# aayush9400/3D-Condtional-Stable-Diffusion

Measured on AMD Instinct MI355X. Metric: latent volumes/sec at 32^3x8ch T=1000 DDPM, higher is better.
Workload: dtype f32 (f16 hi+lo x3 MFMA, f32 accumulate)

## Files before the change

### 3d-condtional-stable-diffusion_amd/csrc/dm3d_conv.hip

```cpp
#include <algorithm>
#include <cstdlib>
#include "dm3d_conv_args.h"
#include <math.h>

namespace {

template <int TD, int TH, int TW, int S, int KS, int WM, int WN>
__global__ __launch_bounds__(256, 2) void conv3d_igemm_f32(const ConvArgs p) {
    constexpr int CK = 16, LDV = CK + 4, NT = 64;
    constexpr int TM = TD * TH * TW;
    constexpr int HD = (TD - 1) * S + KS, HH = (TH - 1) * S + KS, HW = (TW - 1) * S + KS;
    constexpr int HVOX = HD * HH * HW;
    constexpr int TAPS = KS * KS * KS;
    constexpr int MR = TM / WM / 32, NR = NT / WN / 32;
    constexpr int NTHR = WM * WN * 64;
    constexpr int NSLOT = (HVOX * 4 + NTHR - 1) / NTHR;
    static_assert(NTHR == 256, "kernel assumes 4 waves");
    static_assert(TM % (WM * 32) == 0 && NT % (WN * 32) == 0, "tile split");

    extern __shared__ __attribute__((aligned(16))) float smem[];
    float* lds_in = smem;
    float* lds_w = smem + HVOX * LDV;

    const int tid = threadIdx.x;
// ... 97 lines not shown
        for (int tap = 0; tap < TAPS; ++tap) {
            const bool last_tap = tap + 1 == TAPS;
            {
                int nt = tap + 1, nc = c0;
                if (last_tap) { nt = 0; nc = (ch + 1 < p.nchunks) ? c0 + CK : c0; }
                wreg = *reinterpret_cast<const f32x4*>(w_thread + (size_t)nt * w_tap_stride + nc);
            }

            const int kd = tap / (KS * KS), kh = (tap / KS) % KS, kw = tap % KS;
            const int tap_off = ((kd * HH + kh) * HW + kw) * LDV;
            const float* wbuf = lds_w + (tap & 1) * (NT * LDV);
            const float* a_lds[MR];
            const float* b_lds[NR];
#pragma unroll
            for (int mr = 0; mr < MR; ++mr) a_lds[mr] = a_base[mr] + tap_off;
#pragma unroll
            for (int nr = 0; nr < NR; ++nr) b_lds[nr] = wbuf + b_off[nr];
            dm3d_mma_step<MR, NR, CK>(acc, a_lds, b_lds, half);

            if (!last_tap) {
                *reinterpret_cast<f32x4*>(lds_w + ((tap + 1) & 1) * (NT * LDV) + w_lds_off) = wreg;
                __syncthreads();
            }
        }
    }

    const int vrow = p.vec ? (p.vec_idx ? p.vec_idx[b] : b) : 0;
    const size_t sample_elems = (size_t)p.fd * p.fh * p.fw * p.cout;
#pragma unroll
    for (int nr = 0; nr < NR; ++nr) {
        const int n = n0 + wn * (NT / WN) + nr * 32 + l32;
        const bool n_ok = n < p.cout;
        const int nc = n_ok ? n : p.cout - 1;
        float add = p.bias ? p.bias[nc] : 0.0f;
        if (p.vec) add += p.vec[(size_t)vrow * p.vec_ld + nc];
#pragma unroll
        for (int mr = 0; mr < MR; ++mr) {
            size_t o[16];
            bool ok[16];
            float rv[16];
#pragma unroll
            for (int r = 0; r < 16; ++r) {
                const int row = wm * (TM / WM) + mr * 32 + dm3d_acc_row(r, half);
                const int oz = oz0 + row / (TH * TW), oy = oy0 + (row / TW) % TH, ox = ox0 + row % TW;
                ok[r] = n_ok && oz < p.od && oy < p.oh && ox < p.ow;
                o[r] = ok[r] ? ((((size_t)b * p.fd + oz * p.os + ooz) * p.fh + oy * p.os + ooy) * p.fw + ox * p.os + oox) * p.cout + n : 0;
            }
            if (p.res) {
#pragma unroll
                for (int r = 0; r < 16; ++r) rv[r] = p.res[o[r]];
            }
#pragma unroll
            for (int r = 0; r < 16; ++r) {
                float v = acc[mr][nr][r] + add;
                if (p.relu) v = fmaxf(v, 0.0f);
                if (p.prelu) { const float al = p.prelu[o[r] % sample_elems]; v = v > 0.0f ? v : al * v; }
                if (p.res) v += rv[r];
                if (p.relu_out) v = fmaxf(v, 0.0f);
                if (ok[r]) p.out[o[r]] = v;
            }
        }
    }
}

template <int TD, int TH, int TW, int S, int KS, int WM, int WN>
int launch_conv(ConvArgs& a, hipStream_t st) {
    constexpr int LDV = 20;
    constexpr int HVOX = ((TD - 1) * S + KS) * ((TH - 1) * S + KS) * ((TW - 1) * S + KS);
    constexpr size_t lds = (size_t)(HVOX * LDV + 2 * 64 * LDV) * sizeof(float);
    a.bd = (a.od + TD - 1) / TD;
    a.bh = (a.oh + TH - 1) / TH;
    a.bw = (a.ow + TW - 1) / TW;
    static std::atomic<bool> attr_set[64] = {};
    if (int dev = dm3d_dyn_lds(lds, attr_set, "conv", &conv3d_igemm_f32<TD, TH, TW, S, KS, WM, WN>); dev < 0) return dev;
    dim3 grid((unsigned)(a.batch * a.bd * a.bh * a.bw), (unsigned)(a.coutpad / 64), a.parity ? 8u : 1u);
    hipLaunchKernelGGL((conv3d_igemm_f32<TD, TH, TW, S, KS, WM, WN>), grid, dim3(256), lds, st, a);
    return dm3d_launch_check("conv3d_igemm_f32");
}

}


struct ConvKnobs {
    bool pair_off; int ksplit_mode; long split_wgs, split_target; int split_minchunks, split_maxparts; bool wino_split_off;
    int v3_td; long wide_wgs; bool wino_off; int wino_minchunks, wino_split_minchunks;
};
static ConvKnobs conv_knobs() {
    auto num = [](const char* name, long dflt) { const char* e = getenv(name); return e ? atol(e) : dflt; };
    auto zero = [](const char* name) { const char* e = getenv(name); return e && e[0] == '0'; };
    static const ConvKnobs once = {
        zero("DM3D_CONV_PAIR"),
        (int)num("DM3D_CONV_KSPLIT", -1),
        num("DM3D_CONV_SPLIT_WGS", 256),
        num("DM3D_CONV_SPLIT_TARGET", 512),
        (int)num("DM3D_CONV_SPLIT_MINCHUNKS", 2),
        (int)num("DM3D_CONV_SPLIT_MAXPARTS", 16),
        zero("DM3D_CONV_WINO_SPLIT"),
        0, 0, false, 0, 0};
    ConvKnobs k = once;
    k.v3_td = (int)num("DM3D_CONV_V3_TD", 0);
    k.wide_wgs = num("DM3D_CONV_WIDE_WGS", 512);
    k.wino_off = zero("DM3D_CONV_WINO");
    k.wino_minchunks = (int)num("DM3D_CONV_WINO_MINCHUNKS", 2);
    k.wino_split_minchunks = (int)num("DM3D_CONV_WINO_SPLIT_MINCHUNKS", 16);
    return k;
}

static long split_tiles(const ConvArgs& a, int td) {
    return (long)a.batch * ((a.od + td - 1) / td) * ((a.oh + 7) / 8) * ((a.ow + 7) / 8) * (a.coutpad / 64) * (a.parity ? 8 : 1);
}

static int direct_ksplit(const ConvArgs& a, const ConvKnobs& K) {
    const long wgs = split_tiles(a, 4);
    if (K.ksplit_mode == 0 || wgs > K.split_wgs || a.nchunks < 4) return 1;
    int best = 1;
    for (int d = 2; d <= K.split_maxparts; ++d) {
        if (a.nchunks % d != 0 || a.nchunks / d < K.split_minchunks) continue;
        best = d;
        if (wgs * d >= K.split_target) break;
    }
    return best;
}

static int winograd_ksplit(const ConvArgs& a, const ConvKnobs& K) {
    if (K.wino_split_off || a.nchunks % 2 != 0 || a.nchunks < K.wino_split_minchunks) return 1;
    const long wgs = (long)a.batch * (a.od / 8) * (a.oh / 8) * (a.ow / 8) * (a.coutpad / 64);
    return wgs <= 128 ? 2 : 1;
}

static bool winograd_serves(const ConvArgs& a, int which, int ksplit, const ConvKnobs& K) {
    if (!a.wpk_wino || which != DM3D_CONV_K3S1 || a.parity || a.cout <= 32) return false;
    if (a.s_npairs > 0) {
        if (!a.swpk_f) return false;
        const long long svox = (long long)a.batch * a.ind * a.inh * a.inw;
        if (svox * (a.sc1 > a.sc2 ? a.sc1 : a.sc2) * 4 >= (1ll << 32)) return false;
    }
    if (a.od % 8 != 0 || a.oh % 8 != 0 || a.ow % 8 != 0 || a.padz != 1 || a.pady != 1 || a.padx != 1) return false;
    if (K.wino_off || a.nchunks < K.wino_minchunks) return false;
    const long long vox = (long long)a.batch * a.ind * a.inh * a.inw;
    if (vox * (a.c1 > a.c2 ? a.c1 : a.c2) * 4 >= (1ll << 32)) return false;
    const long wgs = (long)a.batch * (a.od / 8) * (a.oh / 8) * (a.ow / 8) * (a.coutpad / 64) * ksplit;
    const long need = K.wide_wgs;
    return wgs >= need || wgs == 256 || (ksplit > 1 && wgs >= (need < 256 ? need : 256L));
}

static int direct_td(const ConvArgs& a, const ConvKnobs& K) {
    if (K.v3_td == 4) return 4;
    if (K.v3_td != 8 && (a.parity || a.s_npairs > 0)) return 4;
    if ((a.out_h2 || a.post_scale) && a.od % 8 != 0) return 4;
    return split_tiles(a, 8) >= K.wide_wgs ? 8 : 4;
}

ConvLaunch dm3d_conv_resolve(const dm3d_conv_desc* d) {
    ConvLaunch r{};
    if (!d) return r;
    const ConvKnobs K = conv_knobs();
    ConvArgs a{};
    a.x1 = d->x1; a.x2 = d->x2; a.c1 = d->c1; a.c2 = d->c2;
    a.ind = d->in_d; a.inh = d->in_h; a.inw = d->in_w;
    const bool par_mode = d->upsample || d->transpose;
    const int cstride = (par_mode || d->stride != 2) ? 1 : 2;
    a.lgd = d->in_d; a.lgh = d->in_h; a.lgw = d->in_w;
    a.od = (d->in_d + cstride - 1) / cstride;
    a.oh = (d->in_h + cstride - 1) / cstride;
    a.ow = (d->in_w + cstride - 1) / cstride;
    a.parity = par_mode ? 1 : 0;
    a.os = par_mode ? 2 : 1;
    a.fd = a.od * a.os; a.fh = a.oh * a.os; a.fw = a.ow * a.os;
    auto pad_front = [&](int in, int out) { int t = (out - 1) * cstride + d->ksize - in; return t > 0 ? t / 2 : 0; };
    a.padz = pad_front(a.lgd, a.od); a.pady = pad_front(a.lgh, a.oh); a.padx = pad_front(a.lgw, a.ow);
    const int cin = d->c1 + d->c2;
    a.cinpad = (int)dm3d_round_up(cin, DM3D_CIN_PAD);
    a.coutpad = (int)dm3d_round_up(d->cout, DM3D_COUT_PAD);
    a.nchunks = a.cinpad / 16;
    a.wpk = d->wpk; a.bias = d->bias; a.pscale = d->pro_scale; a.pshift = d->pro_shift; a.pro_bstride = d->pro_batch_stride;
    a.vec = d->vec; a.vec_idx = d->vec_idx; a.vec_ld = d->vec_ld;
    a.relu = d->relu; a.res = d->res; a.out = d->out; a.cout = d->cout;
    a.prelu = d->prelu_alpha; a.relu_out = d->relu_out;
    a.scratch = d->scratch; a.scratch_bytes = d->scratch_bytes;
    a.split_counters = d->split_counters; a.split_counter_words = d->split_counter_words;
    a.range_flag = d->range_flag; a.range_limit = d->range_limit > 0.0f ? d->range_limit : 65504.0f;
    a.wpk_wino = d->wpk_wino;
    a.x_h2 = d->x1_fmt == DM3D_FMT_H2; a.out_h2 = d->out_fmt == DM3D_FMT_H2;
    a.post_scale = d->post_scale; a.post_shift = d->post_shift;
    if (d->skip_wpk) {
        a.sx1 = d->skip_x1; a.sx2 = d->skip_x2; a.sc1 = d->skip_c1; a.sc2 = d->skip_c2; a.swpk = d->skip_wpk;
        a.s_npairs = (int)(dm3d_round_up(d->skip_c1 + d->skip_c2, 32) / 32);
        a.swpk_f = d->skip_wpk_frag;
    }
    a.batch = d->batch;
    a.out_scale = d->precision == DM3D_PREC_H3 ? ldexpf(1.0f, -d->w_exp) : 1.0f;
    if (par_mode) a.w_parity_stride = d->precision == DM3D_PREC_H3
        ? dm3d_packed_weight_h3_bytes(8, cin, d->cout) / 2 : dm3d_packed_weight_elems(8, cin, d->cout);
    a.gn_stats = d->gn_stats;
    r.a = a;
    r.which = par_mode ? DM3D_CONV_UP
                       : (d->ksize == 1 ? DM3D_CONV_K1 : (d->ksize == 4 ? DM3D_CONV_K4S2 : (d->stride == 2 ? DM3D_CONV_K3S2 : DM3D_CONV_K3S1)));

    if (d->precision != DM3D_PREC_H3) { r.family = DM3D_CONV_FAM_F32; return r; }
    if (dm3d_conv_weight_layout(d->ksize, d->stride, d->upsample, d->transpose, d->cout) != DM3D_WL_PAIR) { r.family = DM3D_CONV_FAM_TAP; return r; }
    const bool wino_geometry = r.which == DM3D_CONV_K3S1 && a.cout > 32 && a.od % 8 == 0 && a.oh % 8 == 0 && a.ow % 8 == 0;
    const int ks_direct = direct_ksplit(a, K), ks_wino = wino_geometry ? winograd_ksplit(a, K) : 1;
    auto bytes = [&](int td, int ks) { return split_tiles(a, td) * ks * (int64_t)(td * 8 * 8 * 64) * (int64_t)sizeof(float); };
    if (winograd_serves(a, r.which, a.split_counters ? ks_wino : 1, K)) {
        r.family = DM3D_CONV_FAM_WINO; r.td = 8; r.nct = 4;
        r.ksplit = a.split_counters ? ks_wino : 1;
    } else {
        r.family = DM3D_CONV_FAM_V3;
        r.nct = (r.which == DM3D_CONV_K3S1 && a.cout <= 32) ? (a.cout <= 16 ? 1 : 2) : 4;
        r.td = r.nct != 4 ? 4 : direct_td(a, K);
        r.ksplit = (r.td == 4 && a.split_counters) ? ks_direct : 1;
    }
    r.tiles = split_tiles(a, r.td);
    r.tile_floats = (long)r.td * 8 * 8 * 64;
    if (r.ksplit > 1) { r.need_words = r.tiles; r.need_bytes = bytes(r.td, r.ksplit); }
    if (d->batch <= 0 || d->cout <= 0 || d->in_d <= 0 || d->in_h <= 0 || d->in_w <= 0) return r;
    if (ks_direct > 1) { r.can_words = split_tiles(a, 4); r.can_bytes = bytes(4, ks_direct); }
    if (ks_wino > 1) { r.can_words = std::max(r.can_words, split_tiles(a, 8)); r.can_bytes = std::max(r.can_bytes, bytes(8, ks_wino)); }
    return r;
}

static int conv_validate(const dm3d_conv_desc* d) {
    DM3D_REQUIRE(d != nullptr, "conv: null descriptor");
    DM3D_REQUIRE(d->x1 && d->wpk && d->out, "conv: x1/wpk/out must be non-null");
    DM3D_REQUIRE(d->ksize == 1 || d->ksize == 3 || (d->ksize == 4 && d->stride == 2), "conv: ksize %d not in {1,3} (4 needs stride 2)", d->ksize);
    DM3D_REQUIRE(d->stride == 1 || d->stride == 2, "conv: stride %d not in {1,2}", d->stride);
    DM3D_REQUIRE(!d->transpose || (d->ksize == 4 && d->stride == 2 && !d->upsample), "conv: transpose needs ksize 4, stride 2, no upsample");
    DM3D_REQUIRE(!(d->upsample && d->stride != 1), "conv: upsample requires stride 1");
    DM3D_REQUIRE(!(d->ksize == 1 && (d->stride != 1 || d->upsample)), "conv: ksize 1 supports stride 1 without upsample only");
    DM3D_REQUIRE(d->batch > 0 && d->in_d > 0 && d->in_h > 0 && d->in_w > 0 && d->cout > 0, "conv: non-positive extent");
    DM3D_REQUIRE(d->c1 > 0 && d->c1 % 4 == 0 && d->c2 >= 0 && d->c2 % 4 == 0, "conv: c1=%d c2=%d must be multiples of 4", d->c1, d->c2);
    DM3D_REQUIRE((d->c2 == 0) == (d->x2 == nullptr), "conv: x2 and c2 must be given together");
    DM3D_REQUIRE(d->c2 == 0 || d->c1 % 16 == 0, "conv: with a second input c1=%d must be a multiple of 16", d->c1);
    DM3D_REQUIRE((d->pro_scale == nullptr) == (d->pro_shift == nullptr), "conv: pro_scale and pro_shift go together");
    DM3D_REQUIRE(!d->vec || d->vec_ld >= d->cout, "conv: vec_ld %d < cout %d", d->vec_ld, d->cout);
    const void* ptrs[] = {d->x1, d->x2, d->wpk, d->pro_scale, d->pro_shift, d->out, d->res};
    for (const void* q : ptrs) DM3D_REQUIRE(dm3d_aligned16(q), "conv: pointer %p is not 16-byte aligned", q);
    const int64_t vox = (int64_t)d->batch * d->in_d * d->in_h * d->in_w;
    DM3D_REQUIRE(vox < (1ll << 31) / 4, "conv: %lld voxels overflow the 32-bit voxel index", (long long)vox);
    DM3D_REQUIRE(d->pro_batch_stride == 0 || (d->pro_batch_stride >= d->c1 + d->c2 && d->pro_batch_stride % 4 == 0),
                 "conv: pro_batch_stride must be 0 or a multiple of 4 >= c1+c2");
    DM3D_REQUIRE((d->split_counters == nullptr) == (d->split_counter_words == 0) && d->split_counter_words >= 0, "conv: split_counters and split_counter_words go together");
    if (d->wpk_wino)
        DM3D_REQUIRE(d->precision == DM3D_PREC_H3 && dm3d_aligned16(d->wpk_wino), "conv: wpk_wino needs precision H3 and 16-byte alignment");
    DM3D_REQUIRE((d->x1_fmt == DM3D_FMT_F32 || d->x1_fmt == DM3D_FMT_H2) && (d->out_fmt == DM3D_FMT_F32 || d->out_fmt == DM3D_FMT_H2),
                 "conv: unknown x1_fmt / out_fmt");
    DM3D_REQUIRE((d->post_scale == nullptr) == (d->post_shift == nullptr), "conv: post_scale and post_shift go together");
    if (d->x1_fmt == DM3D_FMT_H2 || d->out_fmt == DM3D_FMT_H2 || d->post_scale) {
        DM3D_REQUIRE(d->precision == DM3D_PREC_H3 && d->ksize == 3 && d->stride == 1 && !d->upsample && !d->transpose,
                     "conv: x1_fmt / out_fmt / post_* need precision H3, ksize 3, stride 1, no upsample / transpose");
        DM3D_REQUIRE(d->cout > 32 || (d->out_fmt == DM3D_FMT_F32 && !d->post_scale), "conv: out_fmt H2 / post_* need cout > 32");
        DM3D_REQUIRE(d->x1_fmt != DM3D_FMT_H2 || (d->c2 == 0 && d->c1 % 16 == 0 && !d->pro_scale),
                     "conv: an H2 input needs c1 %% 16 == 0, no second input and no prologue");
        DM3D_REQUIRE(d->out_fmt != DM3D_FMT_H2 || (d->in_d % 4 == 0 && d->in_h % 8 == 0 && d->in_w % 8 == 0 && d->cout % 64 == 0 &&
                                                  !d->prelu_alpha),
                     "conv: an H2 output needs extents of whole 4x8x8 bricks and cout %% 64 == 0");
        DM3D_REQUIRE(!d->post_scale || (d->in_d % 4 == 0 && d->in_h % 8 == 0 && d->in_w % 8 == 0 && d->cout % 64 == 0),
                     "conv: post_scale needs extents of whole 4x8x8 bricks and cout %% 64 == 0");
        DM3D_REQUIRE(dm3d_aligned16(d->post_scale) && dm3d_aligned16(d->post_shift), "conv: post_* must be 16-byte aligned");
    }
    if (d->skip_wpk) {
        DM3D_REQUIRE(d->precision == DM3D_PREC_H3 && d->ksize == 3 && d->stride == 1 && !d->upsample && !d->transpose && d->cout > 32,
                     "conv: the fused skip conv needs precision H3, ksize 3, stride 1, no upsample / transpose, cout > 32");
        DM3D_REQUIRE(d->skip_x1 && d->skip_c1 > 0 && d->skip_c1 % 4 == 0 && d->skip_c2 >= 0 && d->skip_c2 % 4 == 0, "conv: skip_c1=%d skip_c2=%d must be multiples of 4", d->skip_c1, d->skip_c2);
        DM3D_REQUIRE((d->skip_c2 == 0) == (d->skip_x2 == nullptr) && (d->skip_c2 == 0 || d->skip_c1 % 16 == 0), "conv: skip_x2 / skip_c2 go together and need skip_c1 %% 16 == 0");
        DM3D_REQUIRE(dm3d_aligned16(d->skip_x1) && dm3d_aligned16(d->skip_x2) && dm3d_aligned16(d->skip_wpk), "conv: skip pointers must be 16-byte aligned");
        DM3D_REQUIRE(dm3d_aligned16(d->skip_wpk_frag), "conv: skip_wpk_frag must be 16-byte aligned");
    }
    DM3D_REQUIRE(dm3d_aligned16(d->scratch) && d->scratch_bytes >= 0, "conv: scratch must be 16-byte aligned");
    DM3D_REQUIRE(d->precision == DM3D_PREC_F32 || d->precision == DM3D_PREC_H3, "conv: unknown precision %d", d->precision);
    DM3D_REQUIRE(d->w_exp >= -100 && d->w_exp <= 100, "conv: w_exp %d out of range", d->w_exp);
    if (d->gn_stats)
        DM3D_REQUIRE(d->out_fmt == DM3D_FMT_F32 && d->cout % 4 == 0 && dm3d_aligned16(d->gn_stats),
                     "conv: gn_stats needs a float32 output, cout %% 4 == 0 and a 16-byte aligned buffer");
    if (d->precision == DM3D_PREC_H3) {
        const int layout = dm3d_conv_weight_layout(d->ksize, d->stride, d->upsample, d->transpose, d->cout);
        DM3D_REQUIRE(d->w_layout == layout, "conv: w_layout %d but this geometry reads layout %d (dm3d_conv_weight_layout)", d->w_layout, layout);
    }
    return DM3D_OK;
}

extern "C" int dm3d_conv3d_ndhwc(const dm3d_conv_desc* d, void* stream) {
    if (int rc = conv_validate(d)) return rc;
    ConvLaunch r = dm3d_conv_resolve(d);
    hipStream_t st = static_cast<hipStream_t>(stream);
    if (r.family == DM3D_CONV_FAM_WINO) return dm3d_conv_launch_h3w(r, st);
    if (r.family == DM3D_CONV_FAM_V3) return dm3d_conv_launch_h3v3(r, st);
    const int rc = r.family == DM3D_CONV_FAM_TAP ? dm3d_conv_launch_h3(r.a, r.which, st) : dm3d_conv_launch_f32(r.a, r.which, st);
    if (rc != DM3D_OK || !r.a.gn_stats) return rc;
    return dm3d_groupnorm_partials(r.a.out, r.a.batch, (int64_t)r.a.fd * r.a.fh * r.a.fw, r.a.cout, r.a.gn_stats, stream);
}

extern "C" int64_t dm3d_packed_weight_skip_h3p_bytes(int32_t cin, int32_t cout) {
    return (cin > 0 && cout > 0) ? dm3d_h3v2_skip_image_bytes(cin, cout) : 0;
// ... 65 lines not shown
```

### 3d-condtional-stable-diffusion_amd/csrc/dm3d_conv_args.h

```cpp
#pragma once
#include "dm3d_common.h"

struct ConvArgs {
    const float* x1; const float* x2; int c1, c2;
    int ind, inh, inw;
    int lgd, lgh, lgw;
    int od, oh, ow;
    int padz, pady, padx;
    int os;
    int ooz, ooy, oox;
    int fd, fh, fw;
    int parity;
    long w_parity_stride;
    const void* wpk; int cinpad, coutpad;
    const float* bias; const float* pscale; const float* pshift; long pro_bstride;
    const float* vec; const int* vec_idx; int vec_ld;
    int relu; const float* res; float* out; int cout;
    const float* prelu; int relu_out;
    int bd, bh, bw;
    int nchunks;
    int batch;
    float out_scale;
    int ksplit;
    int* split_counters;
    int split_counter_words;
    long split_tile_floats;
    void* scratch; long scratch_bytes;
    const float* post_scale; const float* post_shift;
    int out_h2;
    int x_h2;
    const float* sx1; const float* sx2; int sc1, sc2; const void* swpk; int s_npairs;
    const void* swpk_f;
    const void* wpk_wino;
    int* range_flag; float range_limit;
    float* gn_stats;
    int epi_vec4;
};

enum { DM3D_CONV_K3S1 = 0, DM3D_CONV_K3S2 = 1, DM3D_CONV_K1 = 2, DM3D_CONV_UP = 3, DM3D_CONV_K4S2 = 4 };

enum { DM3D_CONV_FAM_F32 = 0,
       DM3D_CONV_FAM_TAP = 1,
       DM3D_CONV_FAM_V3 = 2,
       DM3D_CONV_FAM_WINO = 3 };

struct ConvLaunch {
    ConvArgs a;
    int which;
    int family;
    int td;
    int nct;
    int ksplit;
    long tiles, tile_floats;
    int64_t need_bytes; long need_words;
    int64_t can_bytes; long can_words;
};
ConvLaunch dm3d_conv_resolve(const dm3d_conv_desc* d);

int dm3d_conv_launch_f32(ConvArgs& a, int which, hipStream_t st);
int dm3d_conv_launch_h3(ConvArgs& a, int which, hipStream_t st);
int dm3d_conv_launch_h3v3(const ConvLaunch& r, hipStream_t st);
int dm3d_conv_launch_h3w(const ConvLaunch& r, hipStream_t st);
struct H3v2Launch { ConvArgs k; bool stats_after; };
int dm3d_h3v2_pre_launch(const ConvLaunch& r, H3v2Launch& L);
int dm3d_h3v2_post_launch(const ConvArgs& a, const H3v2Launch& L, hipStream_t st);
int64_t dm3d_h3v2_skip_image_bytes(int cin, int cout);
int dm3d_pack_skip_h3v2(const float* keras_kernel, int cin, int cout, int w_exp, void* packed, hipStream_t st);
int dm3d_pack_skip_h3f(const float* keras_kernel, int cin, int cout, int w_exp, void* packed, hipStream_t st);
int64_t dm3d_h3v2_image_bytes(int taps, int cin, int cout);
int dm3d_pack_h3v2(const float* keras_kernel, int taps, int cin, int cout, int w_exp, const float* in_scale, void* packed, int mode,
                   hipStream_t st);
```

### 3d-condtional-stable-diffusion_amd/csrc/dm3d_conv_h3_host.hip

```cpp
#include "dm3d_conv_h3v2_parts.h"

using namespace h3v2;

int dm3d_h3v2_pre_launch(const ConvLaunch& r, H3v2Launch& L) {
    ConvArgs& k = L.k;
    k = r.a;
    k.bd = (k.od + r.td - 1) / r.td; k.bh = (k.oh + 7) / 8; k.bw = (k.ow + 7) / 8;
    k.ksplit = r.ksplit;
    auto al16 = [](const void* q) { return (reinterpret_cast<size_t>(q) & 15) == 0; };
    k.epi_vec4 = k.cout % 4 == 0 && al16(k.out) && al16(k.bias) && al16(k.res) && al16(k.prelu) && al16(k.post_scale) && al16(k.post_shift)
                 && al16(k.vec) && (k.vec == nullptr || k.vec_ld % 4 == 0);
    k.split_tile_floats = 0;
    if (r.ksplit > 1) {
        k.split_tile_floats = r.tile_floats;
        DM3D_REQUIRE(k.split_counters && k.split_counter_words >= r.need_words, "conv: a Cin-split launch of %ld tiles needs split_counters of as many zeroed words (have %d)",
                     r.tiles, k.split_counter_words);
        DM3D_REQUIRE(k.scratch && (size_t)k.scratch_bytes >= (size_t)r.need_bytes,
                     "conv: scratch of %ld bytes is too small for %d parts x %ld tiles (dm3d_conv_scratch_bytes)", k.scratch_bytes, r.ksplit, r.tiles);
        DM3D_REQUIRE((size_t)r.ksplit * r.tile_floats * sizeof(float) < (1ull << 31), "conv: %d parts overflow a tile's buffer descriptor", r.ksplit);
    }
    L.stats_after = false;
    if (k.gn_stats) {
#ifdef DM3D_EPILOGUE_SCALAR
        const bool fused = false;
#else
        const bool fused = k.od % r.td == 0 && k.oh % 8 == 0 && k.ow % 8 == 0 && k.cout % 64 == 0 && k.epi_vec4 && !k.prelu
                           && !k.out_h2 && !k.post_scale;
#endif
        if (!fused) { k.gn_stats = nullptr; L.stats_after = true; }
    }
    return DM3D_OK;
}

int dm3d_h3v2_post_launch(const ConvArgs& a, const H3v2Launch& L, hipStream_t st) {
    if (L.stats_after) return dm3d_groupnorm_partials(a.out, a.batch, (int64_t)a.fd * a.fh * a.fw, a.cout, a.gn_stats, st);
    return DM3D_OK;
}

namespace {

__global__ __launch_bounds__(256) void pack_weights_h3v2_kernel(const float* __restrict__ w, int taps, int tapsp, int cin, int cout,
                                                                int nchunks, int ntiles, float scale, const float* in_scale,
                                                                _Float16* __restrict__ out, int mode) {
    const long nrec = (long)ntiles * nchunks * tapsp * 64;
    const int npar = (mode == 1 || mode == 2) ? 8 : 1;
    for (long i0 = (long)blockIdx.x * 256 + threadIdx.x; i0 < nrec * 16 * npar; i0 += (long)gridDim.x * 256) {
        const int par = (int)(i0 / (nrec * 16));
        const long i = i0 % (nrec * 16);
        const int k = (int)(i & 15);
        const long rec = i >> 4;
        const int pos = (int)(rec % 64);
        const int tap = (int)((rec / 64) % tapsp);
        const int chunk = (int)((rec / (64L * tapsp)) % nchunks);
        const int nt = (int)(rec / (64L * tapsp * nchunks));
        const int p16 = pos & 15;
        int c = 0;
        for (int cc = 0; cc < 16; ++cc) if (pi_pos(cc) == p16) c = cc;
        const int ci = chunk * 16 + k, co = nt * 64 + (mode == 3 ? 4 * c + (pos >> 4) : (pos & ~15) + c);
        float v = 0.f;
        bool fold = false;
        if (ci < cin && co < cout && tap < taps) {
            if (mode == 3) {
                const int step = tap >> 1, t = step / 5;
                const int tq = (step % 5) < 3 ? (step % 5) * 3 + (tap & 1) : ((step % 5) == 3 ? 2 : ((tap & 1) ? 8 : 5));
                fold = (step % 5) == 3 && (tap & 1);
                {
                    const float g0 = w[((long)(tq * 3 + 0) * cin + ci) * cout + co], g1 = w[((long)(tq * 3 + 1) * cin + ci) * cout + co],
                                g2 = w[((long)(tq * 3 + 2) * cin + ci) * cout + co];
                    v = t == 0 ? g0 : (t == 1 ? 0.5f * ((g0 + g2) + g1) : (t == 2 ? 0.5f * ((g0 + g2) - g1) : g2));
                }
            } else
            v = mode == 1 ? dm3d_up_weight(w, cin, cout, par, tap, ci, co)
              : mode == 2 ? dm3d_convt_weight(w, cin, cout, par, tap, ci, co) : w[((long)tap * cin + ci) * cout + co];
            if (in_scale) v *= in_scale[ci];
            v *= scale;
        }
        const _Float16 hi = (_Float16)v;
        _Float16* r = out + ((long)par * nrec + rec) * REC;
        const int sw = (pos >> 2) & 3;
        r[(((k >> 3) ^ sw) << 3) + (k & 7)] = hi;
        r[(((2 + (k >> 3)) ^ sw) << 3) + (k & 7)] = fold ? (_Float16)0.0f : (_Float16)(v - (float)hi);
    }
}

__global__ __launch_bounds__(256) void pack_skip_h3v2_kernel(const float* __restrict__ w, int cin, int cout, int npairs, int ntiles,
                                                             float scale, _Float16* __restrict__ out) {
    const long nrec = (long)ntiles * npairs * 2 * 64;
    for (long i = (long)blockIdx.x * 256 + threadIdx.x; i < nrec * 16; i += (long)gridDim.x * 256) {
        const int k = (int)(i & 15);
        const long rec = i >> 4;
        const int pos = (int)(rec % 64);
        const int t = (int)((rec / 64) % 2);
        const int pair = (int)((rec / 128) % npairs);
        const int nt = (int)(rec / (128L * npairs));
// ... 67 lines not shown
```

### 3d-condtional-stable-diffusion_amd/csrc/dm3d_conv_h3v3.hip

```cpp
#include "dm3d_conv_h3v2_parts.h"

using namespace h3v2;

#ifdef DM3D_CLOCK_STAMPS
__device__ unsigned long long* g_dbg_stamps_c = nullptr;
extern "C" int dm3d_debug_set_stamps_conv(void* p) { return (int)hipMemcpyToSymbol(HIP_SYMBOL(g_dbg_stamps_c), &p, sizeof(p)); }
#define STAMP(i) do { const unsigned wg_ = blockIdx.x + gridDim.x * blockIdx.y; \
    if (g_dbg_stamps_c && threadIdx.x == 0 && blockIdx.z == 0 && wg_ < 4096) { \
    g_dbg_stamps_c[wg_ * 32 + (i)] = __builtin_amdgcn_s_memtime(); \
    if ((i) == 0) g_dbg_stamps_c[wg_ * 32 + 24] = __builtin_amdgcn_s_memrealtime(); \
    if ((i) == 20) g_dbg_stamps_c[wg_ * 32 + 26] = __builtin_amdgcn_s_memrealtime(); \
    if ((i) == 29) g_dbg_stamps_c[wg_ * 32 + 25] = __builtin_amdgcn_s_memrealtime(); \
    if ((i) == 1) g_dbg_stamps_c[wg_ * 32 + 30] = __builtin_amdgcn_s_memrealtime(); \
    if ((i) == 28) g_dbg_stamps_c[wg_ * 32 + 31] = __builtin_amdgcn_s_memrealtime(); } } while (0)
#else
#define STAMP(i) do { } while (0)
#endif

namespace {

template <int KS, int MODE, int TD, int NCT = 4>
__global__ __launch_bounds__(TD * 64, 2) void conv3d_igemm_h3v3(const ConvArgs p) {
    constexpr int TH = 8, TW = 8, CK = 16, NT = 64, NTHR = TD * 64;
    constexpr int HD = TD - 1 + KS, HH = TH - 1 + KS, HW = TW - 1 + KS, HWP = 12;
// ... 287 lines not shown
                    case 2: __builtin_amdgcn_s_waitcnt(0x0F72); break;
                    case 3: __builtin_amdgcn_s_waitcnt(0x0F73); break;
                    case 4: __builtin_amdgcn_s_waitcnt(0x0F74); break;
                    case 5: __builtin_amdgcn_s_waitcnt(0x0F75); break;
                    case 6: __builtin_amdgcn_s_waitcnt(0x0F76); break;
                    case 7: __builtin_amdgcn_s_waitcnt(0x0F77); break;
                    case 8: __builtin_amdgcn_s_waitcnt(0x0F78); break;
                    case 9: __builtin_amdgcn_s_waitcnt(0x0F79); break;
                    case 10: __builtin_amdgcn_s_waitcnt(0x0F7A); break;
                    default: __builtin_amdgcn_s_waitcnt(0x0F70); break;
                    }
                }
#pragma unroll
                for (int j = (pp - CV0) * SPP; j < (pp - CV0 + 1) * SPP && j < NSLOT; ++j) convert_slot(j);
            }
            __builtin_amdgcn_sched_barrier(0);
            DM3D_PASS(ah, bl);
            __builtin_amdgcn_sched_barrier(0);
            if (last) {
                lds_barrier();
                read_al(0);
                __builtin_amdgcn_sched_barrier(0);
            }
            ws = ws1;
            ++pq;
        }
    }
#undef DM3D_PASS
#undef DM3D_DSR
    STAMP(28);
    asm volatile("s_waitcnt vmcnt(0) lgkmcnt(0)" ::: "memory");
    __builtin_amdgcn_s_barrier();
    asm volatile("" ::: "memory");

    const Brick br = {b, oz0, oy0, ox0, ooz, ooy, oox, ntile, khalf};
    if constexpr (KS == 3 && NCT == 4) {
        skip_phase<TD>(p, smem_v3, acc, br);
    }
    STAMP(19);
    if (p.ksplit > 1) {
        const long tile = ((long)blockIdx.z * gridDim.x + brick_all) * ntiles + ntile;
        const SplitTile stile = split_tile(p, tile, khalf);
        split_store(stile, acc, 0);
        STAMP(20);
        if (!split_is_last(p, tile, reinterpret_cast<unsigned*>(smem_v3))) return;
        STAMP(21);
        split_gather(stile, p, khalf, acc, 0);
        STAMP(22);
    }
    if (p.gn_stats) {
        float gn[NCT * 8];
#pragma unroll
        for (int i = 0; i < NCT * 8; ++i) gn[i] = 0.0f;
        epilogue<TD, NCT>(p, acc, br, -1, 4, -1, gn);
        gn_flush<TD, NCT>(p, gn, br, threadIdx.x >> 6, 1);
    } else {
        epilogue<TD, NCT>(p, acc, br);
    }
    STAMP(29);
}

template <int KS, int MODE, int TD, int NCT = 4>
int launch_v3(const ConvLaunch& r, hipStream_t st) {
    constexpr int HREC = (TD - 1 + KS) * (7 + KS) * 12;
    constexpr int main_halfs = HREC * REC + 4 * 2 * 64 * REC, skip_halfs = (KS == 3 && NCT == 4) ? skip_lds_halfs<TD>() : 0;
    constexpr size_t lds = (size_t)(main_halfs > skip_halfs ? main_halfs : skip_halfs) * sizeof(_Float16);
    static_assert((TD == 4 ? 2 : 1) * lds <= 160 * 1024, "workgroups per CU x LDS");
    static std::atomic<bool> attr_set[64] = {};
    if (int dev = dm3d_dyn_lds(lds, attr_set, "conv", &conv3d_igemm_h3v3<KS, MODE, TD, NCT>); dev < 0) return dev;
    H3v2Launch L;
    if (int rc = dm3d_h3v2_pre_launch(r, L)) return rc;
    const ConvArgs& k = L.k;
    dim3 grid((unsigned)(k.batch * k.bd * k.bh * k.bw), (unsigned)(k.coutpad / 64 * k.ksplit), k.parity ? 8u : 1u);
    hipLaunchKernelGGL((conv3d_igemm_h3v3<KS, MODE, TD, NCT>), grid, dim3(TD * 64), lds, st, k);
    if (int rc = dm3d_launch_check("conv3d_igemm_h3v3")) return rc;
    return dm3d_h3v2_post_launch(r.a, L, st);
}

template <int KS, int MODE>
int launch_td(const ConvLaunch& r, hipStream_t st) {
    if constexpr (KS == 3) {
        if (r.nct != 4) {
            DM3D_REQUIRE(r.a.s_npairs == 0 && !r.a.out_h2, "conv: the fused skip conv / hand-off output need cout > 32");
            return r.nct == 1 ? launch_v3<KS, MODE, 4, 1>(r, st) : launch_v3<KS, MODE, 4, 2>(r, st);
        }
    }
    return r.td == 8 ? launch_v3<KS, MODE, 8>(r, st) : launch_v3<KS, MODE, 4>(r, st);
}

}

int dm3d_conv_launch_h3v3(const ConvLaunch& r, hipStream_t st) {
    const ConvArgs& a = r.a;
    if (r.which == DM3D_CONV_UP) return a.pscale ? launch_td<2, 1>(r, st) : launch_td<2, 0>(r, st);
    if (a.x_h2) return launch_td<3, 2>(r, st);
    return a.pscale ? launch_td<3, 1>(r, st) : launch_td<3, 0>(r, st);
}
```

Measured before the change: 2.363.

## Add persistent narrow-Cout k3 conv kernel with 8-deep bricks and tap-parallel lanes

```diff
diff --git a/3d-condtional-stable-diffusion_amd/csrc/dm3d_conv.hip b/3d-condtional-stable-diffusion_amd/csrc/dm3d_conv.hip
--- a/3d-condtional-stable-diffusion_amd/csrc/dm3d_conv.hip
+++ b/3d-condtional-stable-diffusion_amd/csrc/dm3d_conv.hip
@@ -203,7 +203,7 @@
 
 
 struct ConvKnobs {
-    bool pair_off; int ksplit_mode; long split_wgs, split_target; int split_minchunks, split_maxparts; bool wino_split_off;
+    bool pair_off; int ksplit_mode; long split_wgs, split_target; int split_minchunks, split_maxparts; bool wino_split_off; bool narrow_off;
     int v3_td; long wide_wgs; bool wino_off; int wino_minchunks, wino_split_minchunks;
 };
 static ConvKnobs conv_knobs() {
@@ -217,6 +217,7 @@
         (int)num("DM3D_CONV_SPLIT_MINCHUNKS", 2),
         (int)num("DM3D_CONV_SPLIT_MAXPARTS", 16),
         zero("DM3D_CONV_WINO_SPLIT"),
+        zero("DM3D_CONV_NARROW"),
         0, 0, false, 0, 0};
     ConvKnobs k = once;
     k.v3_td = (int)num("DM3D_CONV_V3_TD", 0);
@@ -331,6 +332,7 @@
         r.nct = (r.which == DM3D_CONV_K3S1 && a.cout <= 32) ? (a.cout <= 16 ? 1 : 2) : 4;
         r.td = r.nct != 4 ? 4 : direct_td(a, K);
         r.ksplit = (r.td == 4 && a.split_counters) ? ks_direct : 1;
+        r.narrow = !K.narrow_off && r.nct != 4 && r.ksplit == 1 && a.s_npairs == 0 && !a.out_h2 && !a.post_scale && !a.prelu && dm3d_h3v2_epi_vec4(a);
     }
     r.tiles = split_tiles(a, r.td);
     r.tile_floats = (long)r.td * 8 * 8 * 64;
diff --git a/3d-condtional-stable-diffusion_amd/csrc/dm3d_conv_args.h b/3d-condtional-stable-diffusion_amd/csrc/dm3d_conv_args.h
--- a/3d-condtional-stable-diffusion_amd/csrc/dm3d_conv_args.h
+++ b/3d-condtional-stable-diffusion_amd/csrc/dm3d_conv_args.h
@@ -51,6 +51,7 @@
     int td;
     int nct;
     int ksplit;
+    bool narrow;
     long tiles, tile_floats;
     int64_t need_bytes; long need_words;
     int64_t can_bytes; long can_words;
@@ -61,6 +62,12 @@
 int dm3d_conv_launch_h3(ConvArgs& a, int which, hipStream_t st);
 int dm3d_conv_launch_h3v3(const ConvLaunch& r, hipStream_t st);
 int dm3d_conv_launch_h3w(const ConvLaunch& r, hipStream_t st);
+int dm3d_conv_launch_h3n(const ConvLaunch& r, hipStream_t st);
+static inline bool dm3d_h3v2_epi_vec4(const ConvArgs& k) {
+    auto al16 = [](const void* q) { return (reinterpret_cast<size_t>(q) & 15) == 0; };
+    return k.cout % 4 == 0 && al16(k.out) && al16(k.bias) && al16(k.res) && al16(k.prelu) && al16(k.post_scale) && al16(k.post_shift)
+           && al16(k.vec) && (k.vec == nullptr || k.vec_ld % 4 == 0);
+}
 struct H3v2Launch { ConvArgs k; bool stats_after; };
 int dm3d_h3v2_pre_launch(const ConvLaunch& r, H3v2Launch& L);
 int dm3d_h3v2_post_launch(const ConvArgs& a, const H3v2Launch& L, hipStream_t st);
diff --git a/3d-condtional-stable-diffusion_amd/csrc/dm3d_conv_h3_host.hip b/3d-condtional-stable-diffusion_amd/csrc/dm3d_conv_h3_host.hip
--- a/3d-condtional-stable-diffusion_amd/csrc/dm3d_conv_h3_host.hip
+++ b/3d-condtional-stable-diffusion_amd/csrc/dm3d_conv_h3_host.hip
@@ -7,9 +7,7 @@
     k = r.a;
     k.bd = (k.od + r.td - 1) / r.td; k.bh = (k.oh + 7) / 8; k.bw = (k.ow + 7) / 8;
     k.ksplit = r.ksplit;
-    auto al16 = [](const void* q) { return (reinterpret_cast<size_t>(q) & 15) == 0; };
-    k.epi_vec4 = k.cout % 4 == 0 && al16(k.out) && al16(k.bias) && al16(k.res) && al16(k.prelu) && al16(k.post_scale) && al16(k.post_shift)
-                 && al16(k.vec) && (k.vec == nullptr || k.vec_ld % 4 == 0);
+    k.epi_vec4 = dm3d_h3v2_epi_vec4(k);
     k.split_tile_floats = 0;
     if (r.ksplit > 1) {
         k.split_tile_floats = r.tile_floats;
diff --git a/3d-condtional-stable-diffusion_amd/csrc/dm3d_conv_h3n.hip b/3d-condtional-stable-diffusion_amd/csrc/dm3d_conv_h3n.hip
--- /dev/null
+++ b/3d-condtional-stable-diffusion_amd/csrc/dm3d_conv_h3n.hip
@@ -0,0 +1,362 @@
+#include "dm3d_conv_h3v2_parts.h"
+
+using namespace h3v2;
+
+namespace {
+
+template <int NCT>
+__device__ __forceinline__ void epilogue_narrow(const ConvArgs& p, f32x4v (&acc)[4][NCT], const int b, const int oz, const int oy0, const int ox0) {
+    const int lane = threadIdx.x & 63, row = lane & 15, g4 = lane >> 4;
+    const int k = row & 3, c4 = row & ~3, dxl = dx_of_row(4 * g4);
+    const bool b0 = (row & 1) != 0, b1 = (row & 2) != 0;
+    auto xor1 = [](float v) { return __builtin_bit_cast(float, __builtin_amdgcn_update_dpp(0, __builtin_bit_cast(int, v), 0xB1, 0xf, 0xf, false)); };
+    auto xor2 = [](float v) { return __builtin_bit_cast(float, __builtin_amdgcn_update_dpp(0, __builtin_bit_cast(int, v), 0x4E, 0xf, 0xf, false)); };
+    const int vrow = p.vec ? (p.vec_idx ? p.vec_idx[b] : b) : 0;
+    const f32x4 zero = {0.f, 0.f, 0.f, 0.f};
+    const size_t zbase = (((size_t)b * p.od + (oz < p.od ? oz : 0)) * p.oh) * p.ow * p.cout;
+    float* const outz = p.out + zbase;
+    const float* const resz = p.res ? p.res + zbase : nullptr;
+    bool ok[4];
+    int off[4];
+#pragma unroll
+    for (int pi = 0; pi < 4; ++pi) {
+        const int y = oy0 + 4 * (pi >> 1) + k, x = ox0 + 4 * (pi & 1) + dxl;
+        ok[pi] = oz < p.od && y < p.oh && x < p.ow;
+        off[pi] = ok[pi] ? (y * p.ow + x) * p.cout + c4 : 0;
+    }
+    f32x4 add_t[NCT];
+    bool n_ok[NCT];
+#pragma unroll
+    for (int ni = 0; ni < NCT; ++ni) {
+        n_ok[ni] = ni * 16 + c4 < p.cout;
+        const int n = n_ok[ni] ? ni * 16 + c4 : 0;
+        add_t[ni] = p.bias ? *reinterpret_cast<const f32x4*>(p.bias + n) : zero;
+        if (p.vec) {
+            const f32x4 vv = *reinterpret_cast<const f32x4*>(p.vec + (size_t)vrow * p.vec_ld + n);
+#pragma unroll
+            for (int j = 0; j < 4; ++j) add_t[ni][j] += vv[j];
+        }
+    }
+    f32x4 rv[4][NCT];
+    if (resz) {
+#pragma unroll
+        for (int pi = 0; pi < 4; ++pi)
+#pragma unroll
+            for (int ni = 0; ni < NCT; ++ni)
+                rv[pi][ni] = *reinterpret_cast<const f32x4*>(resz + (n_ok[ni] ? off[pi] + ni * 16 : 0));
+    }
+    float amax = 0.0f;
+    {
+#pragma unroll
+        for (int pi = 0; pi < 4; ++pi)
+#pragma unroll
+            for (int ni = 0; ni < NCT; ++ni) {
+                float a[4] = {acc[pi][ni][0], acc[pi][ni][1], acc[pi][ni][2], acc[pi][ni][3]};
+                {
+                    float s0 = b0 ? a[0] : a[1], s1 = b0 ? a[2] : a[3];
+                    float r0 = xor1(s0), r1 = xor1(s1);
+                    if (b0) { a[0] = r0; a[2] = r1; } else { a[1] = r0; a[3] = r1; }
+                    s0 = b1 ? a[0] : a[2]; s1 = b1 ? a[1] : a[3];
+                    r0 = xor2(s0); r1 = xor2(s1);
+                    if (b1) { a[0] = r0; a[1] = r1; } else { a[2] = r0; a[3] = r1; }
+                }
+                const bool st = ok[pi] && n_ok[ni];
+                f32x4 v4;
+#pragma unroll
+                for (int j = 0; j < 4; ++j) {
+                    float v = fmaf(a[j], p.out_scale, add_t[ni][j]);
+                    if (p.relu) v = fmaxf(v, 0.0f);
+                    if (resz) v += rv[pi][ni][j];
+                    if (p.relu_out) v = fmaxf(v, 0.0f);
+                    if (st) DM3D_AMAX(amax, v);
+                    v4[j] = v;
+                }
+                if (st) *reinterpret_cast<f32x4*>(outz + off[pi] + ni * 16) = v4;
+            }
+    }
+    if (p.range_flag && amax > p.range_limit) *p.range_flag = 1;
+}
+
+template <int MODE, int NCT, int KQ>
+__global__ __launch_bounds__(256, 2) void conv3d_k3_narrow_h3(const ConvArgs p) {
+    constexpr int TD = 8, TH = 8, TW = 8, CK = 16, NTHR = 256;
+    constexpr int HD = TD + 2, HH = TH + 2, HW = TW + 2, HWP = 12;
+    constexpr int HVOX = HD * HH * HW;
+    constexpr int TAPS = 27, TAPSP = 28;
+    constexpr int NS = TAPSP / KQ;
+    constexpr int PIECES = KQ == 4 ? 1 : 2;
+    constexpr int NSLOT = (HVOX * PIECES + NTHR - 1) / NTHR;
+    constexpr int SPS = (NSLOT + NS - 1) / NS;
+    constexpr int BD = (NCT == 1 || KQ == 4) ? 2 : 1;
+    constexpr int WCHUNK = TAPSP * 64 * REC;
+    static_assert(SPS * NS >= NSLOT && BD < NS, "request schedule");
+
+    extern __shared__ __attribute__((aligned(16))) _Float16 smem_n[];
+    _Float16* lds_in = smem_n;
+
+    const int tid = threadIdx.x;
+    const int lane = tid & 63, wave = tid >> 6;
+    const int row = lane & 15, kg = lane >> 4;
+    const int tsel = KQ == 4 ? kg : kg >> 1;
+    const int q = KQ == 4 ? 0 : kg & 1;
+
+    const int bpv = p.bd * p.bh * p.bw, nbricks = p.batch * bpv;
+    const int G = (int)gridDim.x;
+    int brick = (int)blockIdx.x;
+    if ((G & 7) == 0) brick = ((int)blockIdx.x & 7) * (G >> 3) + ((int)blockIdx.x >> 3);
+    if (brick >= nbricks) return;
+
+    const int piece = KQ == 4 ? 0 : tid & 1;
+    int gv[NSLOT];
+    int pb = 0;
+    auto set_brick = [&](const int br) {
+        const int b = br / bpv, r = br - b * bpv;
+        const int oz0 = (r / (p.bh * p.bw)) * TD, oy0 = ((r / p.bw) % p.bh) * TH, ox0 = (r % p.bw) * TW;
+        pb = b;
+#pragma unroll
+        for (int j = 0; j < NSLOT; ++j) {
+            const int hv = (KQ == 4 ? tid : tid >> 1) + j * (NTHR / PIECES);
+            int g = -1;
+            if (hv < HVOX) {
+                const int hz = hv / (HH * HW), hy = (hv / HW) % HH, hx = hv % HW;
+                const int iz = oz0 - p.padz + hz, iy = oy0 - p.pady + hy, ix = ox0 - p.padx + hx;
+                if (iz >= 0 && iz < p.ind && iy >= 0 && iy < p.inh && ix >= 0 && ix < p.inw)
+                    g = ((b * p.ind + iz) * p.inh + iy) * p.inw + ix;
+            }
+            gv[j] = g;
+        }
+    };
+
+    constexpr bool pro = MODE == 1, xh2 = MODE == 2;
+    f32x4 raw0[NSLOT], raw1[NSLOT];
+    f32x4 sc0 = {1.f, 1.f, 1.f, 1.f}, sc1 = sc0, sh0 = {0.f, 0.f, 0.f, 0.f}, sh1 = sh0;
+    bool ok0 = false, ok1 = false;
+    auto load_halo_slot = [&](const int ch, const int j) {
+        if (xh2) {
+            const char* qp = reinterpret_cast<const char*>(p.x1) + (size_t)ch * 64 + piece * 16 + (size_t)(gv[j] >= 0 ? gv[j] : 0) * ((size_t)p.c1 * 4);
+            raw0[j] = *reinterpret_cast<const f32x4*>(qp);
+            raw1[j] = *reinterpret_cast<const f32x4*>(qp + 32);
+            return;
+        }
+        const int c0 = ch * CK;
+        const float* src;
+        int ldc, cb;
+        if (c0 < p.c1) { src = p.x1; ldc = p.c1; cb = c0; } else { src = p.x2; ldc = p.c2; cb = c0 - p.c1; }
+        const int cpos = cb + piece * 8;
+        const int off0 = cpos < ldc ? cpos : 0, off1 = cpos + 4 < ldc ? cpos + 4 : 0;
+        const float* qp = src + (size_t)(gv[j] >= 0 ? gv[j] : 0) * ldc;
+        raw0[j] = *reinterpret_cast<const f32x4*>(qp + off0);
+        raw1[j] = *reinterpret_cast<const f32x4*>(qp + off1);
+    };
+    auto load_chunk_params = [&](const int ch) {
+        if (xh2) return;
+        const int c0 = ch * CK;
+        const int ldc = c0 < p.c1 ? p.c1 : p.c2, cpos = (c0 < p.c1 ? c0 : c0 - p.c1) + piece * 8;
+        ok0 = cpos < ldc;
+        ok1 = cpos + 4 < ldc;
+        if (pro) {
+            const int s0 = ok0 ? c0 + piece * 8 : 0, s1 = ok1 ? c0 + piece * 8 + 4 : 0;
+            const size_t bo = (size_t)pb * p.pro_bstride;
+            sc0 = *reinterpret_cast<const f32x4*>(p.pscale + bo + s0);
+            sh0 = *reinterpret_cast<const f32x4*>(p.pshift + bo + s0);
+            sc1 = *reinterpret_cast<const f32x4*>(p.pscale + bo + s1);
+            sh1 = *reinterpret_cast<const f32x4*>(p.pshift + bo + s1);
+        }
+    };
+    auto convert_slot = [&](const int j) {
+        const bool in = gv[j] >= 0;
+        h8 shi_j, slo_j;
+        f32x4 v0 = raw0[j], v1 = raw1[j];
+        if (pro) {
+#pragma unroll
+            for (int e = 0; e < 4; ++e) {
+                v0[e] = dm3d_silu(fmaf(v0[e], sc0[e], sh0[e]));
+                v1[e] = dm3d_silu(fmaf(v1[e], sc1[e], sh1[e]));
+            }
+        }
+        if (xh2) {
+            const f32x4 z = {0.f, 0.f, 0.f, 0.f};
+            shi_j = __builtin_bit_cast(h8, in ? v0 : z);
+            slo_j = __builtin_bit_cast(h8, in ? v1 : z);
+        } else {
+            split8(v0, v1, (in && ok0) ? 65504.0f : 0.0f, (in && ok1) ? 65504.0f : 0.0f, shi_j, slo_j);
+        }
+        raw0[j] = __builtin_bit_cast(f32x4, shi_j);
+        raw1[j] = __builtin_bit_cast(f32x4, slo_j);
+    };
+    auto store_image = [&]() {
+#pragma unroll
+        for (int j = 0; j < NSLOT; ++j) {
+            const int hv = (KQ == 4 ? tid : tid >> 1) + j * (NTHR / PIECES);
+            if (hv < HVOX) {
+                const int v = (hv / HW) * HWP + hv % HW;
+                const int o = v * REC + ((piece ^ swz(v)) << 3);
+                *reinterpret_cast<f32x4*>(lds_in + o) = raw0[j];
+                *reinterpret_cast<f32x4*>(lds_in + (o ^ 16)) = raw1[j];
+            }
+        }
+    };
+
+    const _Float16* const wbase = static_cast<const _Float16*>(p.wpk);
+    const int b_pos = pi_pos(row);
+    const int b_lane = (tsel * 64 + b_pos) * REC + ((q ^ swz(b_pos)) << 3);
+    h8 bqh[BD][NCT], bql[BD][NCT];
+    auto load_b = [&](const int ch, const int s, h8 (&bh)[NCT], h8 (&bl)[NCT]) {
+        const _Float16* wp = wbase + (size_t)ch * WCHUNK + s * (KQ * 64 * REC);
+#pragma unroll
+        for (int ni = 0; ni < NCT; ++ni) {
+            bh[ni] = *reinterpret_cast<const h8*>(wp + ni * 16 * REC + b_lane);
+            bl[ni] = *reinterpret_cast<const h8*>(wp + ni * 16 * REC + (b_lane ^ 16));
+        }
+    };
+
+    int a_rec = ((wave * 2) * HH + (row & 3)) * HWP + dx_of_row(row);
+    auto tap_rec = [](const int t) { const int tc = t < TAPS ? t : TAPS - 1; return ((tc / 9) * HH + (tc / 3) % 3) * HWP + tc % 3; };
+
+    auto a_offs = [&](const int s, const int z, int& o0, int& o1) {
+        int rsel;
+        if constexpr (KQ == 4) {
+            const int r01 = (kg & 1) ? tap_rec(4 * s + 1) : tap_rec(4 * s), r23 = (kg & 1) ? tap_rec(4 * s + 3) : tap_rec(4 * s + 2);
+            rsel = (kg & 2) ? r23 : r01;
+        } else {
+            rsel = tsel ? tap_rec(2 * s + 1) : tap_rec(2 * s);
+        }
+        const int v0 = a_rec + z * (HH * HWP) + rsel, v1 = v0 + 4;
+        o0 = v0 * REC + ((q ^ swz(v0)) << 3);
+        o1 = v1 * REC + ((q ^ swz(v1)) << 3);
+    };
+    auto read_frag = [&](h8 (&f)[4], const int o0, const int o1) {
+#pragma unroll
+        for (int py = 0; py < 2; ++py) {
+            f[py * 2 + 0] = *reinterpret_cast<const h8*>(lds_in + o0 + py * (48 * REC));
+            f[py * 2 + 1] = *reinterpret_cast<const h8*>(lds_in + o1 + py * (48 * REC));
+        }
+    };
+
+    f32x4v acc[2][4][NCT];
+    auto zero_acc = [&]() {
+#pragma unroll
+        for (int z = 0; z < 2; ++z)
+#pragma unroll
+            for (int pi = 0; pi < 4; ++pi)
+#pragma unroll
+                for (int ni = 0; ni < NCT; ++ni) acc[z][pi][ni] = f32x4v{0.f, 0.f, 0.f, 0.f};
+    };
+    zero_acc();
+
+    set_brick(brick);
+#pragma unroll
+    for (int i = 0; i < BD; ++i) load_b(0, i, bqh[i], bql[i]);
+#pragma unroll
+    for (int j = 0; j < NSLOT; ++j) load_halo_slot(0, j);
+    load_chunk_params(0);
+
+    for (;;) {
+        const int b = brick / bpv, rb = brick - b * bpv;
+        const int oz0 = (rb / (p.bh * p.bw)) * TD, oy0 = ((rb / p.bw) % p.bh) * TH, ox0 = (rb % p.bw) * TW;
+        const bool more = brick + G < nbricks;
+        for (int ch = 0; ch < p.nchunks; ++ch) {
+            asm volatile("" : "+v"(a_rec));
+#pragma unroll
+            for (int j = 0; j < NSLOT; ++j) convert_slot(j);
+            __syncthreads();
+            store_image();
+            __syncthreads();
+            const bool wrap = ch + 1 == p.nchunks;
+            const int ch_next = wrap ? 0 : ch + 1;
+            if (wrap && more) set_brick(brick + G);
+            h8 al[4];
+#pragma unroll
+            for (int s = 0; s < NS; ++s) {
+#pragma unroll
+                for (int j = s * SPS; j < (s + 1) * SPS && j < NSLOT; ++j) load_halo_slot(ch_next, j);
+                if (s == 0) load_chunk_params(ch_next);
+                h8 nbh[NCT], nbl[NCT];
+                if (s + BD < NS) load_b(ch, s + BD, nbh, nbl); else load_b(ch_next, s + BD - NS, nbh, nbl);
+#define DM3D_NPASS(A, B)                                                                                                   \
+                    _Pragma("unroll") for (int pi = 0; pi < 4; ++pi)                                                      \
+                        _Pragma("unroll") for (int ni = 0; ni < NCT; ++ni)                                                \
+                            acc[z][pi][ni] = __builtin_amdgcn_mfma_f32_16x16x32_f16(A[pi], B[ni], acc[z][pi][ni], 0, 0, 0)
+#pragma unroll
+                for (int z = 0; z < 2; ++z) {
+                    h8 ah[4];
+                    int o0, o1;
+                    a_offs(s, z, o0, o1);
+                    if (s == 0 && z == 0) read_frag(al, o0 ^ 16, o1 ^ 16);
+                    read_frag(ah, o0, o1);
+                    DM3D_NPASS(al, bqh[0]);
+                    __builtin_amdgcn_sched_barrier(0);
+                    if (z == 0 || s + 1 < NS) {
+                        a_offs(z == 0 ? s : s + 1, z ^ 1, o0, o1);
+                        read_frag(al, o0 ^ 16, o1 ^ 16);
+                    }
+                    DM3D_NPASS(ah, bqh[0]);
+                    DM3D_NPASS(ah, bql[0]);
+                    __builtin_amdgcn_sched_barrier(0);
+                }
+#undef DM3D_NPASS
+#pragma unroll
+                for (int i = 0; i + 1 < BD; ++i)
+#pragma unroll
+                    for (int ni = 0; ni < NCT; ++ni) { bqh[i][ni] = bqh[i + 1][ni]; bql[i][ni] = bql[i + 1][ni]; }
+#pragma unroll
+                for (int ni = 0; ni < NCT; ++ni) { bqh[BD - 1][ni] = nbh[ni]; bql[BD - 1][ni] = nbl[ni]; }
+                __builtin_amdgcn_sched_barrier(0);
+            }
+        }
+        epilogue_narrow<NCT>(p, acc[0], b, oz0 + wave * 2, oy0, ox0);
+        epilogue_narrow<NCT>(p, acc[1], b, oz0 + wave * 2 + 1, oy0, ox0);
+        if (!more) break;
+        brick += G;
+        zero_acc();
+    }
+}
+
+template <int MODE, int NCT, int KQ>
+int launch_n(const ConvLaunch& r, hipStream_t st) {
+    constexpr size_t lds = (size_t)(10 * 10 * 12 * REC) * sizeof(_Float16);
+    static_assert(2 * lds <= 160 * 1024, "two workgroups per CU");
+    static std::atomic<bool> attr_set[64] = {};
+    static std::atomic<int> cus[64] = {};
+    const int dev = dm3d_dyn_lds(lds, attr_set, "conv", &conv3d_k3_narrow_h3<MODE, NCT, KQ>);
+    if (dev < 0) return dev;
+    if (cus[dev].load(std::memory_order_acquire) == 0) {
+        int n = 0;
+        DM3D_HIP(hipDeviceGetAttribute(&n, hipDeviceAttributeMultiprocessorCount, dev));
+        cus[dev].store(n > 0 ? n : 256, std::memory_order_release);
+    }
+    const int ncu = cus[dev].load(std::memory_order_relaxed);
+    H3v2Launch L;
+    if (int rc = dm3d_h3v2_pre_launch(r, L)) return rc;
+    ConvArgs& k = L.k;
+    DM3D_REQUIRE(k.epi_vec4 && !k.prelu, "conv: the narrow form needs 16-byte aligned epilogue operands and no PReLU");
+    k.bd = (k.od + 7) / 8;
+    const long bricks = (long)k.batch * k.bd * k.bh * k.bw;
+    long g = bricks;
+    if (bricks > 2L * ncu) g = ncu >= 4 ? 2L * ncu / 8 * 8 : 2L * ncu;
+    if (const char* cap = getenv("DM3D_CONV_NARROW_GRID"); cap && atol(cap) > 0 && atol(cap) < g) g = atol(cap);
+    if (g < 1) g = 1;
+    hipLaunchKernelGGL((conv3d_k3_narrow_h3<MODE, NCT, KQ>), dim3((unsigned)g), dim3(256), lds, st, k);
+    if (int rc = dm3d_launch_check("conv3d_k3_narrow_h3")) return rc;
+    return dm3d_h3v2_post_launch(r.a, L, st);
+}
+
+template <int MODE>
+int launch_n_mode(const ConvLaunch& r, hipStream_t st) {
+    const ConvArgs& a = r.a;
+    if constexpr (MODE != 2) {
+        if (a.c2 == 0 && a.c1 <= 8) return r.nct == 1 ? launch_n<MODE, 1, 4>(r, st) : launch_n<MODE, 2, 4>(r, st);
+    }
+    return r.nct == 1 ? launch_n<MODE, 1, 2>(r, st) : launch_n<MODE, 2, 2>(r, st);
+}
+
+}
+
+int dm3d_conv_launch_h3n(const ConvLaunch& r, hipStream_t st) {
+    const ConvArgs& a = r.a;
+    DM3D_REQUIRE(r.narrow && r.which == DM3D_CONV_K3S1 && (r.nct == 1 || r.nct == 2) && r.ksplit == 1 && a.coutpad == 64 && !a.parity
+                 && a.s_npairs == 0 && !a.out_h2 && !a.post_scale && a.nchunks >= 1,
+                 "conv: the narrow form serves k3 / stride 1, cout <= 32, no Cin split, no fused skip, float32 output");
+    if (a.x_h2) return launch_n_mode<2>(r, st);
+    return a.pscale ? launch_n_mode<1>(r, st) : launch_n_mode<0>(r, st);
+}
diff --git a/3d-condtional-stable-diffusion_amd/csrc/dm3d_conv_h3v3.hip b/3d-condtional-stable-diffusion_amd/csrc/dm3d_conv_h3v3.hip
--- a/3d-condtional-stable-diffusion_amd/csrc/dm3d_conv_h3v3.hip
+++ b/3d-condtional-stable-diffusion_amd/csrc/dm3d_conv_h3v3.hip
@@ -393,6 +393,7 @@
     if constexpr (KS == 3) {
         if (r.nct != 4) {
             DM3D_REQUIRE(r.a.s_npairs == 0 && !r.a.out_h2, "conv: the fused skip conv / hand-off output need cout > 32");
+            if (r.narrow) return dm3d_conv_launch_h3n(r, st);
             return r.nct == 1 ? launch_v3<KS, MODE, 4, 1>(r, st) : launch_v3<KS, MODE, 4, 2>(r, st);
         }
     }
```

Result: no change. 2.368 (median of 3 runs) (+0.2%).
